# jwwangchn/BONAI

Measured on AMD Instinct MI355X. Metric: training img/s at 1024x1024 LOFT R50-FPN, higher is better.
Workload: dtype bf16; 1 GPU; LOFT R50-FPN + FOA, 8x1024x1024 synthetic tiles per GPU (BASELINE configs[1]), 80 gt/img, full train step (fwd+losses+bwd+allreduce+clip+SGD), random-init weights, RoI heads at the load of a trained RPN (first proposals = jittered gt boxes); global_batch=8, per_gpu_batch=8, parallelism=dp1, graph_features=False

## Files before the change

### bonai_amd/csrc/elementwise.hip

```cpp
#include "loft_common.h"
#include "../../include/loft_hip.h"
#include "conv_tap.h"

__device__ __forceinline__ void ld8(const bf16_t* p, float v[8]) {
    uint4 t = *reinterpret_cast<const uint4*>(p);
    unpack8_16(t, v);
}
__device__ __forceinline__ void st8(bf16_t* p, const float v[8]) {
    *reinterpret_cast<uint4*>(p) = pack8_16(v);
}

__device__ __forceinline__ void ld8(const float* p, float v[8]) { ld4(p, v); ld4(p + 4, v + 4); }
__device__ __forceinline__ void st8(float* p, const float v[8]) { st4(p, v); st4(p + 4, v + 4); }

static inline dim3 ew_grid(long nvec) {
    long b = (nvec + 255) / 256;
    if (b > 8192) b = 8192;
    if (b < 1) b = 1;
    return dim3((unsigned)b);
}

__global__ void relu_bwd_kernel(const bf16_t* __restrict__ g, const bf16_t* __restrict__ y, bf16_t* __restrict__ out,
                                long nvec) {
    for (long i = blockIdx.x * (long)blockDim.x + threadIdx.x; i < nvec; i += (long)gridDim.x * blockDim.x) {
// ... 851 lines not shown
                    for (int k = 0; k < 4; ++k) q[k] = (uint32_t)tp[(2 * k) * ldw] | ((uint32_t)tp[(2 * k + 1) * ldw] << 16);
                    *reinterpret_cast<uint4*>(wpt + ((long)t * CinP + c0 + ccl) * CoutP + nn) = make_uint4(q[0], q[1], q[2], q[3]);
                }
            }
        } else if (wpt) {
            const int hsh = ntsh - 1, hp = 1 << hsh;
            for (int i = threadIdx.x; i < RS * 64 * hp; i += 256) {
                const int np = i & (hp - 1), r2 = i >> hsh, ccl = r2 & 63, t = r2 >> 6;
                const int nn = n0 + 2 * np, cc = c0 + ccl;
                if (nn < CoutP && cc < CinP) {
                    const bf16_t* tp = bt + 2 * np * ldw + ccl * RS + t;
                    *reinterpret_cast<uint32_t*>(wpt + ((long)t * CinP + cc) * CoutP + nn) = (uint32_t)tp[0] | ((uint32_t)tp[ldw] << 16);
                }
            }
        }
    }
}
LOFT_EXPORT int loft_fold_pack_multi(const int64_t* desc, int n, int64_t nchunks, void* stream) {
    if (n <= 0 || nchunks <= 0) return 0;
    long blocks = nchunks < 16384 ? nchunks : 16384;
    hipLaunchKernelGGL(fold_pack_multi_kernel, dim3((unsigned)blocks), dim3(256), 0, (hipStream_t)stream, (const long*)desc, n,
                       (long)nchunks);
    LOFT_LAUNCH_CHECK();
    return 0;
}

__global__ __launch_bounds__(256) void transpose_bf16_kernel(const bf16_t* __restrict__ src, bf16_t* __restrict__ dst, int R, int Cc) {
    __shared__ bf16_t t[64][66];
    const int r0 = blockIdx.y * 64, c0 = blockIdx.x * 64;
    for (int i = threadIdx.x; i < 64 * 32; i += 256) {
        const int r = i >> 5, cp = (i & 31) * 2;
        uint32_t v = 0;
        if (r0 + r < R && c0 + cp < Cc) v = *reinterpret_cast<const uint32_t*>(src + (long)(r0 + r) * Cc + c0 + cp);
        t[r][cp] = (bf16_t)(v & 0xffff);
        t[r][cp + 1] = (bf16_t)(v >> 16);
    }
    __syncthreads();
    for (int i = threadIdx.x; i < 64 * 32; i += 256) {
        const int c = i >> 5, rp = (i & 31) * 2;
        if (c0 + c < Cc && r0 + rp < R)
            *reinterpret_cast<uint32_t*>(dst + (long)(c0 + c) * R + r0 + rp) = (uint32_t)t[rp][c] | ((uint32_t)t[rp + 1][c] << 16);
    }
}
LOFT_EXPORT int loft_transpose_bf16(const void* src, void* dst, int R, int Cc, void* stream) {
    if (R <= 0 || Cc <= 0) return 0;
    if ((R & 1) || (Cc & 1)) return (int)hipErrorInvalidValue;
    hipLaunchKernelGGL(transpose_bf16_kernel, dim3(loft_cdiv(Cc, 64), loft_cdiv(R, 64)), dim3(256), 0, (hipStream_t)stream,
                       (const bf16_t*)src, (bf16_t*)dst, R, Cc);
    LOFT_LAUNCH_CHECK();
    return 0;
}

__global__ __launch_bounds__(256) void fold_unpack_bwd_kernel(const float* __restrict__ dwp, const float* __restrict__ db,
                                                              const float* __restrict__ w, const float* __restrict__ gamma,
                                                              const float* __restrict__ mean, const float* __restrict__ var,
                                                              float eps, int Cout, int Cin, int RS, float* __restrict__ dw,
                                                              float* __restrict__ dgamma, float* __restrict__ dbeta, int CoutP,
                                                              int CinP, int accumulate) {
    const int n = blockIdx.x;
    const float rs = gamma ? rsqrtf(var[n] + eps) : 1.f;
    const float scale = gamma ? gamma[n] * rs : 1.f;
    float acc = 0.f;
    const int per = Cin * RS;
    for (int j = threadIdx.x; j < per; j += blockDim.x) {
        const int c = j / RS, t = j - c * RS;
        const float g = dwp[((long)t * CoutP + n) * CinP + c];
        const long wi = (long)n * per + j;
        if (dw) dw[wi] = (accumulate ? dw[wi] : 0.f) + g * scale;
        if (gamma) acc += g * w[wi];
    }
    if (gamma) {
        for (int o = 32; o > 0; o >>= 1) acc += __shfl_down(acc, o, 64);
        __shared__ float part[4];
        if ((threadIdx.x & 63) == 0) part[threadIdx.x >> 6] = acc;
        __syncthreads();
        if (threadIdx.x == 0) {
            const float s = part[0] + part[1] + part[2] + part[3];
            const float dbn = db ? db[n] : 0.f;
            if (dgamma) dgamma[n] = (accumulate ? dgamma[n] : 0.f) + (s * rs - dbn * mean[n] * rs);
            if (dbeta) dbeta[n] = (accumulate ? dbeta[n] : 0.f) + dbn;
        }
    }
}
__global__ __launch_bounds__(256) void fold_unpack_bwd_multi_kernel(const long* __restrict__ desc, int njobs, int lds_floats) {
    const int lo = find_record(desc, njobs, (long)blockIdx.x);
    const long* d = desc + (long)lo * 16;
    const float* dwp = reinterpret_cast<const float*>(d[0]);
    const float* db = reinterpret_cast<const float*>(d[1]);
    const float* w = reinterpret_cast<const float*>(d[2]);
    const float* gamma = reinterpret_cast<const float*>(d[3]);
    const float* mean = reinterpret_cast<const float*>(d[4]);
    const float* var = reinterpret_cast<const float*>(d[5]);
    float* dw = reinterpret_cast<float*>(d[6]);
    float* dgamma = reinterpret_cast<float*>(d[7]);
    float* dbeta = reinterpret_cast<float*>(d[8]);
    const float eps = __int_as_float((int)(d[9] & 0xffffffffl));
    const int nsp = (int)(d[9] >> 32) > 1 ? (int)(d[9] >> 32) : 1;
    const int Cin = (int)d[11], CoutP = (int)d[13], CinP = (int)d[14];
    const bool nmajor = d[12] < 0;
    const int RS = (int)(nmajor ? -d[12] : d[12]);
    const int n = (int)(blockIdx.x - d[15]);
    const long sps = (long)RS * CoutP * CinP;
    auto ld1 = [&](const float* p) {
        float v = *p;
        int q = 1;
        for (; q + 3 < nsp; q += 4) {
            const float u0 = p[q * sps], u1 = p[(q + 1) * sps], u2 = p[(q + 2) * sps], u3 = p[(q + 3) * sps];
            v += (u0 + u1) + (u2 + u3);
        }
        for (; q < nsp; ++q) v += p[q * sps];
        return v;
    };
    auto ld4s = [&](const float* p) {
        float4 v = *reinterpret_cast<const float4*>(p);
        int q = 1;
        for (; q + 3 < nsp; q += 4) {
            const float4 u0 = *reinterpret_cast<const float4*>(p + q * sps), u1 = *reinterpret_cast<const float4*>(p + (q + 1) * sps);
            const float4 u2 = *reinterpret_cast<const float4*>(p + (q + 2) * sps), u3 = *reinterpret_cast<const float4*>(p + (q + 3) * sps);
            v.x += (u0.x + u1.x) + (u2.x + u3.x); v.y += (u0.y + u1.y) + (u2.y + u3.y);
            v.z += (u0.z + u1.z) + (u2.z + u3.z); v.w += (u0.w + u1.w) + (u2.w + u3.w);
        }
        for (; q < nsp; ++q) {
            const float4 u = *reinterpret_cast<const float4*>(p + q * sps);
            v.x += u.x; v.y += u.y; v.z += u.z; v.w += u.w;
        }
        return v;
    };
    const float rs = gamma ? rsqrtf(var[n] + eps) : 1.f;
    const float scale = gamma ? gamma[n] * rs : 1.f;
    float acc = 0.f;
    const int per = Cin * RS;
    if (nmajor) {
        extern __shared__ float urow[];
        const int CB = min(Cin, lds_floats / RS);
        const unsigned cb_mul = CB == 1 ? 0u : 0xFFFFFFFFu / (unsigned)CB + 1u;
        for (int cb0 = 0; cb0 < Cin; cb0 += CB) {
            const int cbn = min(CB, Cin - cb0), cnt = cbn * RS;
            const bool small = CB * RS < 65536 && cbn == CB;
            __syncthreads();
            for (int j = threadIdx.x; j < cnt; j += blockDim.x) {
                const int t = cbn == 1 ? j : (small ? (int)__umulhi((unsigned)j, cb_mul) : j / cbn), c = j - t * cbn;
                urow[c * RS + t] = ld1(dwp + (long)n * per + (long)t * CinP + cb0 + c);
            }
            __syncthreads();
            for (int j = threadIdx.x; j < cnt; j += blockDim.x) {
                const long wi = (long)n * per + (long)cb0 * RS + j;
                if (dw) dw[wi] += urow[j] * scale;
            }
        }
        if (threadIdx.x == 0 && dbeta && db) dbeta[n] += db[n];
        return;
    }
    if (RS > 1 && per <= lds_floats) {
        extern __shared__ float urow[];
        if ((Cin & 3) == 0 && (CinP & 3) == 0) {
            for (int j = threadIdx.x * 4; j < per; j += blockDim.x * 4) {
                const int t = j / Cin, c = j - t * Cin;
                const float4 v = ld4s(dwp + ((long)t * CoutP + n) * CinP + c);
                urow[c * RS + t] = v.x; urow[(c + 1) * RS + t] = v.y; urow[(c + 2) * RS + t] = v.z; urow[(c + 3) * RS + t] = v.w;
            }
            __syncthreads();
            for (int j = threadIdx.x * 4; j < per; j += blockDim.x * 4) {
                const float4 g = *reinterpret_cast<const float4*>(urow + j);
                const long wi = (long)n * per + j;
                if (dw) {
                    float4 o = *reinterpret_cast<float4*>(dw + wi);
                    o.x += g.x * scale; o.y += g.y * scale; o.z += g.z * scale; o.w += g.w * scale;
                    *reinterpret_cast<float4*>(dw + wi) = o;
                }
                if (gamma) {
                    const float4 ww = *reinterpret_cast<const float4*>(w + wi);
                    acc += g.x * ww.x + g.y * ww.y + g.z * ww.z + g.w * ww.w;
                }
            }
        } else {
            for (int j = threadIdx.x; j < per; j += blockDim.x) {
                const int t = j / Cin, c = j - t * Cin;
                urow[c * RS + t] = ld1(dwp + ((long)t * CoutP + n) * CinP + c);
            }
            __syncthreads();
            for (int j = threadIdx.x; j < per; j += blockDim.x) {
                const float g = urow[j];
                const long wi = (long)n * per + j;
                if (dw) dw[wi] += g * scale;
                if (gamma) acc += g * w[wi];
            }
        }
    } else if (RS == 1 && (Cin & 3) == 0 && (CinP & 3) == 0) {
        for (int j = threadIdx.x * 4; j < per; j += blockDim.x * 4) {
            const float4 g = ld4s(dwp + (long)n * CinP + j);
            const long wi = (long)n * per + j;
            if (dw) {
                float4 o = *reinterpret_cast<float4*>(dw + wi);
                o.x += g.x * scale; o.y += g.y * scale; o.z += g.z * scale; o.w += g.w * scale;
                *reinterpret_cast<float4*>(dw + wi) = o;
            }
            if (gamma) {
                const float4 ww = *reinterpret_cast<const float4*>(w + wi);
                acc += g.x * ww.x + g.y * ww.y + g.z * ww.z + g.w * ww.w;
            }
        }
    } else
    for (int j = threadIdx.x; j < per; j += blockDim.x) {
        const int c = j / RS, t = j - c * RS;
        const float g = ld1(dwp + ((long)t * CoutP + n) * CinP + c);
        const long wi = (long)n * per + j;
        if (dw) dw[wi] += g * scale;
        if (gamma) acc += g * w[wi];
    }
    if (gamma) {
        for (int o = 32; o > 0; o >>= 1) acc += __shfl_down(acc, o, 64);
        __shared__ float part[4];
        if ((threadIdx.x & 63) == 0) part[threadIdx.x >> 6] = acc;
        __syncthreads();
        if (threadIdx.x == 0) {
            const float s = part[0] + part[1] + part[2] + part[3];
            const float dbn = db ? db[n] : 0.f;
            if (dgamma) dgamma[n] += s * rs - dbn * mean[n] * rs;
            if (dbeta) dbeta[n] += dbn;
        }
    } else if (threadIdx.x == 0 && dbeta && db) {
        dbeta[n] += db[n];
    }
}
LOFT_EXPORT int loft_fold_unpack_bwd_multi(const int64_t* desc, int njobs, int64_t nblocks, int lds_floats, void* stream) {
    if (njobs <= 0 || nblocks <= 0) return 0;
    if (lds_floats < 0 || lds_floats > 16384) return (int)hipErrorInvalidValue;
    hipLaunchKernelGGL(fold_unpack_bwd_multi_kernel, dim3((unsigned)nblocks), dim3(256), (size_t)lds_floats * 4, (hipStream_t)stream,
                       (const long*)desc, njobs, lds_floats);
    LOFT_LAUNCH_CHECK();
    return 0;
}
LOFT_EXPORT int loft_fold_unpack_bwd(const float* dwp, const float* db, const float* w, const float* gamma, const float* mean,
                                     const float* var, float eps, int Cout, int Cin, int RS, float* dw, float* dgamma,
                                     float* dbeta, int CoutP, int CinP, int accumulate, void* stream) {
    if (Cout <= 0) return 0;
    if (CoutP < Cout || CinP < Cin) return (int)hipErrorInvalidValue;
    hipLaunchKernelGGL(fold_unpack_bwd_kernel, dim3(Cout), dim3(256), 0, (hipStream_t)stream, dwp, db, w, gamma, mean, var, eps,
                       Cout, Cin, RS, dw, dgamma, dbeta, CoutP, CinP, accumulate);
    LOFT_LAUNCH_CHECK();
    return 0;
}

template <typename T, int V> struct NhbIO;
template <> struct NhbIO<bf16_t, 4> {
    static __device__ __forceinline__ void ld(const bf16_t* p, float* v) { ld4(p, v); }
    static __device__ __forceinline__ void st(bf16_t* p, const float* v) { st4(p, v); }
};
template <> struct NhbIO<bf16_t, 8> {
    static __device__ __forceinline__ void ld(const bf16_t* p, float* v) { ld8(p, v); }
    static __device__ __forceinline__ void st(bf16_t* p, const float* v) { st8(p, v); }
};
template <> struct NhbIO<float, 4> {
    static __device__ __forceinline__ void ld(const float* p, float* v) {
        const float4 a = *reinterpret_cast<const float4*>(p);
        v[0] = a.x; v[1] = a.y; v[2] = a.z; v[3] = a.w;
    }
    static __device__ __forceinline__ void st(float* p, const float* v) { *reinterpret_cast<float4*>(p) = make_float4(v[0], v[1], v[2], v[3]); }
};

template <int NOUT, int V, typename XT = bf16_t>
__global__ __launch_bounds__(256) void narrow_head_bwd_kernel(const float* __restrict__ g, int gs, const XT* __restrict__ x,
                                                              const float* __restrict__ w, long M, int Cin, int relu_in,
                                                              XT* __restrict__ gx, float* __restrict__ dw,
                                                              float* __restrict__ db) {
    const int cg = Cin / V;
    const int ppi = 256 / cg > 0 ? 256 / cg : 1;
    const int tid = threadIdx.x;
    const int col = tid % cg, sub = tid / cg;
    const bool act = sub < ppi;
    const int c0 = col * V;
    float wr[NOUT][V], acc[NOUT][V], bacc[NOUT];
#pragma unroll
    for (int n = 0; n < NOUT; ++n) {
#pragma unroll
        for (int q = 0; q < V; ++q) { wr[n][q] = w[(long)n * Cin + c0 + q]; acc[n][q] = 0.f; }
        bacc[n] = 0.f;
    }
    if (act) {
        constexpr int UN = 4;
        const long step = ppi;
        const long per_blk = ((M + gridDim.x - 1) / gridDim.x + (long)ppi * UN - 1) / ((long)ppi * UN) * ((long)ppi * UN);
        const long m_beg = (long)blockIdx.x * per_blk, m_end = m_beg + per_blk < M ? m_beg + per_blk : M;
        for (long m0 = m_beg + sub; m0 < m_end; m0 += step * UN) {
            float xv[UN][V], gv[UN][NOUT];
#pragma unroll
            for (int u = 0; u < UN; ++u) {
                const long m = m0 + u * step;
                if (m < m_end) {
                    NhbIO<XT, V>::ld(x + m * Cin + c0, xv[u]);
#pragma unroll
                    for (int n = 0; n < NOUT; ++n) gv[u][n] = g[m * gs + n];
                } else {
#pragma unroll
                    for (int q = 0; q < V; ++q) xv[u][q] = 0.f;
#pragma unroll
                    for (int n = 0; n < NOUT; ++n) gv[u][n] = 0.f;
                }
            }
#pragma unroll
            for (int u = 0; u < UN; ++u) {
                const long m = m0 + u * step;
                float o[V];
#pragma unroll
                for (int q = 0; q < V; ++q) o[q] = 0.f;
// ... 183 lines not shown
```

### bonai_amd/debug.py

```python
import contextlib
import os

SWITCHES = {
    'no_side_stream': 'mask / bbox branches, the RPN proposal chain and the backbone weight gradients all on the main stream '
                      '(the mode of bench.py\'s roofline instrumentation)',
    'no_bbox_side_stream': 'the bbox head on the main stream (the mask branch keeps its side stream)',
    'no_rpn_side_stream': 'the RPN proposal chain (sort, decode, NMS) on the main stream',
    'no_rpn_target_prefetch': 'RPN anchor assignment + sampling after the RPN convs on the main stream, not beside the backbone',
    'no_rpn_loss_stream': 'the RPN losses (and with them the sparse RPN backward) on the main stream',
    'no_wgrad_stream': 'backbone weight-gradient launches on the data-gradient stream',
    'unpack_stream': 'the batched weight-gradient unpack launches (descriptor upload + loft_fold_unpack_bwd_multi) on a stream of their '
                     'own instead of on the main stream between the data-gradient kernels (round 6: measured, not the default)',
    'no_prepack': 'BN fold + operand packing per conv per step instead of one launch per step (kernels.PrepackRegistry)',
    'no_unpack_queue': 'one loft_fold_unpack_bwd launch per conv instead of the batched unpack (kernels.UnpackQueue)',
    'no_grad_sink': 'gradients returned to autograd and accumulated by it, not deposited in the arena by the kernels',
    'no_leaf_sink': 'narrow heads and the sparse RPN backward return their parameter gradients to autograd (per-parameter accumulation '
                    'launches) instead of depositing them through the unpack queue (nn._queue_param_grads)',
    'no_head_fusion': 'narrow 1x1 heads (RPN objectness + deltas, mask logits) as launches of their own instead of in the producing '
                      'conv\'s epilogue (loft_conv_tap_bf16_head)',
    'no_grad_join': 'autograd sums the two data gradients of a backbone stage output (next stage + FPN lateral) with an elementwise add '
                    'instead of the residual block taking the lateral\'s deposit as its data-gradient residual (nn.JOIN)',
    'no_deconv_fusion': 'the mask head\'s 2x2 deconvolution as four parity launches instead of one launch whose four channel tiles are '
                        'the four taps (loft_deconv2x2_bf16: the input tile read once)',
    'no_zero_pool': 'torch.zeros / torch.empty per accumulation buffer instead of the step\'s pre-zeroed / scratch slabs',
    'no_feat_hub': 'autograd sums the RPN / RoI-extractor gradients of the FPN maps (no shared per-level gradient map)',
    'no_block_fusion': 'one autograd node per conv of a residual block instead of nn.res_block',
    'no_linear_fn': 'Linear layers through the generic conv node',
    'no_bneck_fusion': 'the frozen / inference 64-plane bottleneck as three (four) tap-conv launches instead of conv1 + the fused tail '
                       '(loft_bneck_tail_bf16: 3x3 + 1x1 expansion + shortcut + ReLU in one launch)',
    'no_pair_fusion': 'the last 1x1 of bottleneck k and the first 1x1 of bottleneck k+1 (layer2 / layer3) as two launches each way instead '
                      'of one (loft_bneck_pair_bf16: the block output is written once and not re-read as the next conv1\'s operand)',
    'wgrad_no_patch': 'the tap weight-gradient kernel for 64-channel high-resolution layers (no patch kernel)',
    'roi_fp32_bwd': 'RoIAlign backward into fp32 maps + a cast',
    'roi_sort': 'RoIAlign forward workgroups in (image, level, row strip) launch order for lists of >= 256 RoIs (loft_roi_order; '
                'measured neutral on the step, not shipped)',
    'no_roi_sort': 'list (sampling) order even where kernels.ROI_FWD_SORT_MIN asks for the launch order',
    'narrow_mfma_bwd': 'narrow (<= 8 output) heads backward as padded MFMA GEMMs',
}


class _Switches:
    __slots__ = tuple(SWITCHES)

    def __init__(self):
        for k in SWITCHES:
            setattr(self, k, bool(os.environ.get('LOFT_' + k.upper())))

    def active(self):
        return sorted(k for k in SWITCHES if getattr(self, k))

    @contextlib.contextmanager
    def override(self, **kw):
        prev = {k: getattr(self, k) for k in kw}
        try:
            for k, v in kw.items():
                setattr(self, k, bool(v))
            yield self
        finally:
            for k, v in prev.items():
                setattr(self, k, v)


DBG = _Switches()
```

### bonai_amd/engine.py

```python
import os

import torch
import torch.distributed as dist

from . import kernels as K
from .debug import DBG


class FlatArena:

    def __init__(self, model):
        self.params = [p for p in model.parameters() if p.requires_grad]
        dev = self.params[0].device
        order = list(reversed(self.params))
        self.offsets, off = {}, 0
        for p in order:
            self.offsets[id(p)] = off
            off += (p.numel() + 7) // 8 * 8
        self.numel = off
        self.data = torch.zeros(off, dtype=torch.float32, device=dev)
        self.grad = torch.zeros(off, dtype=torch.float32, device=dev)
        self.momentum = torch.zeros(off, dtype=torch.float32, device=dev)
        for p in order:
            o = self.offsets[id(p)]
# ... 144 lines not shown
        for raw, st in producers.items():
            ev = self._events.get((bi, raw))
            if ev is None:
                ev = self._events[(bi, raw)] = torch.cuda.Event()
            ev.record(st)
            self.stream.wait_event(ev)
        with torch.cuda.stream(self.stream):
            self.works.append(dist.all_reduce(view, async_op=True))

    def finish(self):
        if not self.enabled:
            return
        while self._next < len(self.buckets):
            self._launch(self._next)
            self._next += 1
        if self.on_gpu and self.measure:
            e0 = torch.cuda.Event(enable_timing=True)
            e0.record(torch.cuda.current_stream())
        if self.on_gpu:
            if self.works and dist.get_backend() == 'nccl':
                with torch.cuda.stream(self.stream):
                    self.works[-1].wait()
            else:
                for w in self.works:
                    w.wait()
            if self.measure:
                e1 = torch.cuda.Event(enable_timing=True)
                e1.record(self.stream)
                self.exposed.append((e0, e1))
            torch.cuda.current_stream().wait_stream(self.stream)
        else:
            for w in self.works:
                w.wait()
        self._prune()

    def _prune(self):
        if not self.prune_hooks or self.capturing:
            return
        for p in self.arena.order:
            k = id(p)
            if k in self._via_sink:
                if k in self._hooks:
                    self._sunk_streak[k] += 1
                    if self._sunk_streak[k] >= self.PRUNE_AFTER:
                        self._hooks.pop(k).remove()
            elif k in self._hooks:
                self._sunk_streak[k] = 0
            elif k not in self._seen:
                self._arm(p)

    def exposed_ms(self):
        ev, self.exposed = self.exposed, []
        if not ev:
            return None
        return sum(max(0.0, a.elapsed_time(b)) for a, b in ev) / len(ev)


def step_lr(base_lr, it, epoch, warmup_iters=300, warmup_ratio=0.001, steps=(16, 22), gamma=0.1, step=None):
    if step is not None:
        steps = step
    lr = base_lr * gamma ** sum(epoch >= s for s in steps)
    if it < warmup_iters:
        k = (1 - it / warmup_iters) * (1 - warmup_ratio)
        lr = lr * (1 - k)
    return lr


class Trainer:
    def __init__(self, model, lr=0.005, momentum=0.9, weight_decay=1e-4, max_norm=35.0, bucket_bytes=25 << 20,
                 loss_scale=1.0, graph_features=False):
        self.model = model
        self.graph_features = bool(graph_features)
        self._fgraphs = None
        self._unpack_stream = None
        self._steps_run = 0
        self.lr, self.mu, self.wd, self.max_norm = lr, momentum, weight_decay, max_norm
        self.loss_scale = float(loss_scale)
        self.arena = FlatArena(model)
        self.reducer = BucketedAllReduce(self.arena, bucket_bytes)
        self.world = dist.get_world_size() if self.reducer.enabled else 1
        self.gnorm_sq = torch.zeros(1, dtype=torch.float32, device=self.arena.data.device)
        self.iter = 0
        self.prepack = K.PrepackRegistry()
        self._sink = self.reducer._sink if self.reducer.enabled else (lambda p: None)

    def _graph_step_setup(self, img):
        from .graphs import FeatureGraphs
        fg = self._fgraphs
        if fg is None:
            fg = self._fgraphs = FeatureGraphs(self)
        if fg.ready and fg.validate() is not None:
            import warnings
            warnings.warn(f'hipGraphs of backbone + neck dropped and recaptured: {fg.stale}', RuntimeWarning)
        if not fg.ready and fg.failed is None and self._steps_run >= 2 and self.prepack.order:
            self.reducer.capturing = True
            try:
                fg.capture(img)
            except Exception as e:
                import warnings
                fg.failed = f'{type(e).__name__}: {e}'
                warnings.warn(f'hipGraph capture of backbone + neck failed, the trainer stays on eager launches: {fg.failed}',
                              RuntimeWarning)
            finally:
                self.reducer.capturing = False
        if fg.ready:
            self.model.feat_provider = fg.provider

    def optimizer_state_dict(self):
        a = self.arena
        state, idx = {}, {}
        for i, p in enumerate(self.model.parameters()):
            idx[id(p)] = i
        if self.iter > 0:
            for p in a.params:
                o = a.offsets[id(p)]
                state[idx[id(p)]] = dict(momentum_buffer=a.momentum[o:o + p.numel()].view(p.shape).detach().cpu().clone())
        group = dict(lr=self.lr, momentum=self.mu, dampening=0, weight_decay=self.wd, nesterov=False,
                     params=list(range(len(idx))))
        return dict(state=state, param_groups=[group], iter=self.iter, sampler_calls=int(K._SAMPLE_CALLS[0]))

    def load_optimizer_state(self, sd):
        a = self.arena
        params = list(self.model.parameters())
        state = sd.get('state', {})
        groups = sd.get('param_groups')
        if groups and sum(len(g.get('params', ())) for g in groups) != len(params):
            raise RuntimeError(f"optimizer state covers {sum(len(g['params']) for g in groups)} parameters, the model has "
                               f'{len(params)}: it was written for a different model')
        todo = []
        for i, st in state.items():
            if not 0 <= int(i) < len(params):
                raise RuntimeError(f'optimizer state index {i} outside the model\'s {len(params)} parameters')
            p = params[int(i)]
            buf = st.get('momentum_buffer')
            if buf is None:
                continue
            if tuple(buf.shape) != tuple(p.shape):
                raise RuntimeError(f'optimizer state {i}: momentum_buffer {tuple(buf.shape)} does not fit parameter '
                                   f'{tuple(p.shape)} (parameter order differs from the checkpoint\'s)')
            if id(p) in a.offsets:
                todo.append((a.offsets[id(p)], p.numel(), buf))
        for o, n, buf in todo:
            a.momentum[o:o + n].copy_(buf.reshape(-1).to(a.momentum.device))
        self.iter = int(sd.get('iter', self.iter))
        if 'sampler_calls' in sd:
            K._SAMPLE_CALLS[0] = int(sd['sampler_calls'])

    def train_step(self, data, lr=None):
        self.arena.grad.zero_()
        self.arena.rebind_grads()
        self.reducer.begin()
        for p in self.arena.params:
            p._loft_pending = 0
            p._loft_sunk = False
        from . import nn as F2
        prev_pp, prev_wpl = F2.PREPACK, K.WEIGHT_PLANES
        if self.arena.data.is_cuda and not DBG.no_prepack:
            F2.PREPACK = self.prepack
            K.WEIGHT_PLANES = self.prepack.wplanes
            self.prepack.run(self.iter)
        prev_hub = F2.HUB_ENABLED
        F2.HUB_ENABLED = self.arena.data.is_cuda and not DBG.no_feat_hub
        F2.JOIN = {} if (self.arena.data.is_cuda and not DBG.no_grad_join) else None
        F2.PAIR_G.clear()
        if self.graph_features and self.arena.data.is_cuda and K.PROFILE is None and F2.PREPACK is not None \
                and hasattr(self.model, 'extract_feat'):
            self._graph_step_setup(data['img'])
        try:
            out = self.model.train_step(data)
        except BaseException:
            F2.JOIN = None
            K.WEIGHT_PLANES = prev_wpl
            raise
        finally:
            F2.PREPACK = prev_pp
            F2.HUB_ENABLED = prev_hub
            if self.graph_features:
                self.model.feat_provider = None
        prev, F2.GRAD_SINK = F2.GRAD_SINK, (self._sink if self.arena.data.is_cuda and not DBG.no_grad_sink else None)
        if self.arena.data.is_cuda and not DBG.no_zero_pool:
            K.zero_pool_begin(self.arena.data.device)
        if F2.GRAD_SINK is not None and not DBG.no_unpack_queue:
            ustream = None
            if DBG.unpack_stream and not DBG.no_side_stream:
                if getattr(self, '_unpack_stream', None) is None:
                    self._unpack_stream = torch.cuda.Stream()
                ustream = self._unpack_stream
            lim = int(os.environ.get('LOFT_UNPACK_LIMIT', '0')) or (24 if self.reducer.enabled else 48)
            note = self.reducer.note_queued if (self.reducer.enabled and os.environ.get('LOFT_NO_NOTE_FLUSH') != '1') else None
            F2.UNPACK_Q = K.UnpackQueue(limit=lim, note=note, stream=ustream)
            if not DBG.no_side_stream and not DBG.no_wgrad_stream:
                if getattr(self, '_wgrad_stream', None) is None:
                    self._wgrad_stream = torch.cuda.Stream()
                F2.WGRAD_STREAM = self._wgrad_stream
        try:
            (out['loss'] if self.loss_scale == 1.0 else out['loss'] * self.loss_scale).backward()
            if F2.UNPACK_Q is not None:
                F2.UNPACK_Q.flush()
        finally:
            if F2.UNPACK_Q is not None:
                F2.UNPACK_Q.join()
            F2.UNPACK_Q = None
            F2.WGRAD_STREAM = None
            F2.GRAD_SINK = prev
            F2.HUB = None
            F2.JOIN = None
            K.WEIGHT_PLANES = prev_wpl
            K.zero_pool_end()
        self.reducer.finish()
        self.gnorm_sq.zero_()
        K.sumsq_(self.arena.grad, self.gnorm_sq)
        K.sgd_momentum_(self.arena.data, self.arena.grad, self.arena.momentum, self.gnorm_sq, self.max_norm,
                        self.lr if lr is None else lr, self.mu, self.wd, grad_scale=1.0 / (self.world * self.loss_scale))
        self.iter += 1
        self._steps_run += 1
        return out
```

### bonai_amd/kernels.py

```python
import ctypes
import os

import numpy as np
import torch

from . import lib as L
from .debug import DBG as _DBG

c_int, c_int64, c_float, c_void_p = ctypes.c_int, ctypes.c_int64, ctypes.c_float, ctypes.c_void_p


def h2d(values, dtype, device):
    t = torch.from_numpy(values).to(dtype) if isinstance(values, np.ndarray) else torch.tensor(values, dtype=dtype)
    if torch.device(device).type != 'cuda':
        return t.to(device)
    if H2D_KEEP is not None:
        global _H2D_STREAM
        for _ in range(64):
            if _H2D_STREAM is None:
                _H2D_STREAM = torch.cuda.Stream()
            with torch.cuda.stream(_H2D_STREAM):
                if not torch.cuda.is_current_stream_capturing():
                    break
            _H2D_STREAM = None
# ... 1894 lines not shown
    nv = nval.contiguous().view(torch.uint8) if nval.dtype == torch.bool else nval.contiguous()
    tab = torch.empty(4, B, dtype=torch.int32, device=dev)
    L.check(lib.loft_roi_sample_offsets(L.ptr(pv), L.ptr(nv), B, P, Q, L.ptr(tab), L.stream()), 'loft_roi_sample_offsets')
    Mx, Nx = B * (P + Q), B * P
    out = dict(rois=torch.zeros(Mx, 5, device=dev), labels=torch.empty(Mx, dtype=torch.int64, device=dev),
               label_weights=torch.empty(Mx, device=dev), bbox_targets=torch.empty(Mx, 4, device=dev),
               bbox_weights=torch.empty(Mx, 4, device=dev), pos_rois=torch.empty(Nx, 5, device=dev),
               pos_b=torch.empty(Nx, dtype=torch.int64, device=dev), pos_gt_i=torch.empty(Nx, dtype=torch.int64, device=dev),
               pos_sel=torch.empty(Nx, dtype=torch.int64, device=dev))
    if Mx > 0:
        L.check(lib.loft_roi_sample_targets(L.ptr(cand.float().contiguous()), Ncand, L.ptr(gt_inds.contiguous()),
                                            L.ptr(gts.float().contiguous()), L.ptr(gt_labels.contiguous()), int(gts.shape[1]),
                                            L.ptr(pidx.contiguous()), L.ptr(nidx.contiguous()), P, Q, B, L.ptr(tab[0]), L.ptr(tab[1]),
                                            L.ptr(tab[2]), L.ptr(tab[3]), int(num_classes), L.arr(c_float, list(means)),
                                            L.arr(c_float, list(stds)), L.ptr(out['rois']), L.ptr(out['labels']),
                                            L.ptr(out['label_weights']), L.ptr(out['bbox_targets']), L.ptr(out['bbox_weights']),
                                            L.ptr(out['pos_rois']), L.ptr(out['pos_b']), L.ptr(out['pos_gt_i']), L.ptr(out['pos_sel']),
                                            L.stream()), 'loft_roi_sample_targets')
    host = torch.empty(2, B, dtype=torch.int32, pin_memory=True)
    host.copy_(tab[:2], non_blocking=True)
    ev = torch.cuda.Event()
    ev.record()
    return _RoiTargets(out, host, ev, B, Mx if num_expected is None else min(Mx, B * int(num_expected)))


def roi_sample_targets(cand, gt_inds, gts, gt_labels, pidx, pval, nidx, nval, num_classes, means, stds):
    return roi_sample_targets_begin(cand, gt_inds, gts, gt_labels, pidx, pval, nidx, nval, num_classes, means, stds).finish()


_SAMPLE_CALLS = [0]


def random_sample(gt_inds, num, max_pos, mode='random'):
    lib = L.load()
    L.dev_check(gt_inds)
    gt_inds = gt_inds.contiguous()
    if gt_inds.dtype != torch.int64:
        raise L.LoftHipError(f'gt_inds must be int64, got {gt_inds.dtype}')
    B, N = gt_inds.shape
    P, Q = min(int(max_pos), N), min(int(num), N)
    dev = gt_inds.device
    pidx = torch.empty(B, P, dtype=torch.int64, device=dev)
    nidx = torch.empty(B, Q, dtype=torch.int64, device=dev)
    pval = torch.empty(B, P, dtype=torch.uint8, device=dev)
    nval = torch.empty(B, Q, dtype=torch.uint8, device=dev)
    _SAMPLE_CALLS[0] += 1
    seed = (torch.initial_seed() * 6364136223846793005 + _SAMPLE_CALLS[0] * 1442695040888963407) & 0xFFFFFFFFFFFFFFFF
    if B > 0 and N > 0:
        ws = torch.empty(B * ((N + 15) // 16 * 16), dtype=torch.uint8, device=dev)
        L.check(lib.loft_random_sample(L.ptr(gt_inds), B, N, int(num), int(max_pos), 0 if mode == 'first' else 1,
                                       ctypes.c_uint64(seed), L.ptr(pidx), L.ptr(pval), L.ptr(nidx), L.ptr(nval), L.ptr(ws),
                                       L.stream()), 'loft_random_sample')
    return pidx, pval.view(torch.bool), nidx, nval.view(torch.bool)


def sampled_avg_factor(pos_valid, neg_valid):
    lib = L.load()
    L.dev_check(pos_valid, neg_valid)
    pv, nv = pos_valid.contiguous().view(torch.uint8), neg_valid.contiguous().view(torch.uint8)
    out = torch.empty(1, dtype=torch.float32, device=pv.device)
    L.check(lib.loft_sampled_avg_factor(L.ptr(pv), L.ptr(nv), int(pv.shape[0]), int(pv.shape[1]), int(nv.shape[1]), L.ptr(out),
                                        L.stream()), 'loft_sampled_avg_factor')
    return out


def narrow_head_bwd(g, x, w, relu_in=False, need_gx=True, need_dw=True, need_db=True):
    lib = L.load()
    L.dev_check(g, x, w)
    x = _nhwc(x)
    g = g.float().contiguous(memory_format=torch.channels_last)
    N, Cin, H, W = x.shape
    Cout = w.shape[0]
    w2 = w.reshape(Cout, Cin).float().contiguous()
    f32 = x.dtype == torch.float32
    gx = empty_nhwc(N, Cin, H, W, torch.float32 if f32 else L.act16(), x.device) if need_gx else None
    dw = pooled_zeros((Cout, Cin), x.device) if need_dw else None
    db = pooled_zeros((Cout,), x.device) if need_db else None
    fn = lib.loft_narrow_head_bwd_f32 if f32 else lib.loft_narrow_head_bwd
    L.check(fn(L.ptr(g), int(g.shape[1]), L.ptr(x), L.ptr(w2), c_int64(N * H * W), Cin, Cout, int(relu_in),
               L.ptr(gx), L.ptr(dw), L.ptr(db), L.stream()), 'loft_narrow_head_bwd')
    return gx, dw, db


class UnpackQueue:

    def __init__(self, limit=48, note=None, stream=None):
        self.limit = limit
        self.note = note
        self.jobs, self.done = [], []
        self.main = torch.cuda.current_stream() if torch.cuda.is_available() else None
        self.main_raw = L.stream().value if self.main is not None else None
        self.home = stream if stream is not None else self.main
        self.home_raw = self.home.cuda_stream if stream is not None else self.main_raw
        self.dedicated = stream is not None
        self.events = []
        self.main_jobs = False
        self.keep = []
        self._targets = set()

    def add(self, dwp, db, w, bn, eps, slots, on_done=(), flat_chw=None, nsplit=1, params=()):
        tgt = slots[0].data_ptr() if slots[0] is not None else None
        if tgt is not None:
            if tgt in self._targets:
                if os.environ.get('LOFT_DEBUG_TARGETS'):
                    print('unpack queue: slot used twice in one batch ->', tuple(w.shape), 'jobs pending', len(self.jobs), flush=True)
                self.flush()
            self._targets.add(tgt)
        self.jobs.append((dwp, db, w, bn, float(eps), slots, flat_chw, int(nsplit)))
        if self.home is not None:
            raw = L.stream().value
            if raw == self.home_raw:
                pass
            elif self.dedicated and raw == self.main_raw:
                self.main_jobs = True
            else:
                ev = torch.cuda.Event()
                ev.record()
                self.events.append(ev)
                if not self.dedicated:
                    for t in (dwp, db):
                        if t is not None:
                            t.record_stream(self.home)
            if self.dedicated:
                self.keep.append((dwp, db))
        self.done.extend(on_done)
        if len(self.jobs) >= self.limit or (self.note is not None and self.note(params)):
            self.flush()

    def join(self, stream=None):
        if self.dedicated:
            (stream or self.main).wait_stream(self.home)
        self.keep = []

    def flush(self):
        if self.home is not None and L.stream().value != self.home_raw:
            if self.main_jobs:
                ev = torch.cuda.Event()
                ev.record(self.main)
                self.events.append(ev)
                self.main_jobs = False
            with torch.cuda.stream(self.home):
                return self.flush()
        for ev in self.events:
            self.home.wait_event(ev)
        self.events = []
        if self.jobs:
            import struct
            rows, blk = [], 0
            p = lambda t: 0 if t is None else t.data_ptr()
            for dwp, db, w, bn, eps, (dw, dg, dbeta), flat, nsplit in self.jobs:
                if flat is not None:
                    Cout, Cin, RS = w.shape[0], flat[0], -(flat[1] * flat[2])
                    coutp, cinp = Cout, Cin
                else:
                    Cout, Cin = w.shape[0], w.shape[1]
                    RS = w.shape[2] * w.shape[3] if w.dim() == 4 else 1
                    coutp, cinp = dwp.shape[-2], dwp.shape[-1]
                g, _, m, v = bn if bn is not None else (None, None, None, None)
                rows.append([p(dwp), p(db), p(w), p(g), p(m), p(v), p(dw), p(dg), p(dbeta),
                             (struct.unpack('<I', struct.pack('<f', eps))[0]) | (nsplit << 32), Cout, Cin, RS, coutp, cinp, blk])
                blk += Cout
            desc = h2d(rows, torch.int64, self.jobs[0][2].device)
            lds = max([min(r[11], 64) * abs(r[12]) if r[12] < 0 else r[11] * r[12] for r in rows
                       if r[12] < 0 or (r[12] > 1 and r[11] * r[12] <= 16384)], default=0)
            if lds > 16384:
                raise L.LoftHipError(f'fold_unpack_bwd_multi: a record needs {lds} floats of LDS')
            L.check(L.load().loft_fold_unpack_bwd_multi(L.ptr(desc), len(rows), c_int64(blk), int(lds), L.stream()),
                    'loft_fold_unpack_bwd_multi')
            self.jobs = []
            self._targets = set()
        done, self.done = self.done, []
        for f in done:
            f()


def fold_unpack_bwd(dwp, db, w, bn=None, eps=1e-5, need_dw=True, out=None):
    lib = L.load()
    w = w.contiguous()
    Cout, Cin, R, S = w.shape
    dev = w.device
    g = m = v = dg = dbeta = None
    if out is not None:
        dw, dg, dbeta = out
        if bn is not None:
            g, _, m, v = [t.contiguous() for t in bn]
    else:
        dw = torch.empty_like(w) if need_dw else None
        if bn is not None:
            g, _, m, v = [t.contiguous() for t in bn]
            dg = torch.empty(Cout, dtype=torch.float32, device=dev)
            dbeta = torch.empty(Cout, dtype=torch.float32, device=dev)
    L.check(lib.loft_fold_unpack_bwd(L.ptr(dwp), L.ptr(db), L.ptr(w), L.ptr(g), L.ptr(m), L.ptr(v), c_float(eps), Cout, Cin,
                                     R * S, L.ptr(dw), L.ptr(dg), L.ptr(dbeta), dwp.shape[-2], dwp.shape[-1], int(out is not None),
                                     L.stream()),
            'loft_fold_unpack_bwd')
    return dw, dg, dbeta
```

Baseline: 231.6 img/s.

## Store first weight-gradient deposit instead of zeroing the whole gradient arena

Adds a DepositPlan that learns which gradient-arena slots the batched unpack kernel writes each step. On later steps it zeroes only the gaps, and the kernel's first deposit into a covered slot overwrites instead of read-modify-write accumulating. This removes the full arena memset and one read per weight gradient element. It also vectorises the n-major unpack path with float4 loads and stores. The cost is host-side bookkeeping per deposit and a correctness dependence on the deposit order staying the same between steps.

```diff
diff --git a/bonai_amd/csrc/elementwise.hip b/bonai_amd/csrc/elementwise.hip
--- a/bonai_amd/csrc/elementwise.hip
+++ b/bonai_amd/csrc/elementwise.hip
@@ -957,6 +957,7 @@
         }
     }
 }
+constexpr int UNPACK_STORE_W = 60, UNPACK_STORE_G = 61, UNPACK_STORE_B = 62;
 __global__ __launch_bounds__(256) void fold_unpack_bwd_multi_kernel(const long* __restrict__ desc, int njobs, int lds_floats) {
     const int lo = find_record(desc, njobs, (long)blockIdx.x);
     const long* d = desc + (long)lo * 16;
@@ -970,7 +971,9 @@
     float* dgamma = reinterpret_cast<float*>(d[7]);
     float* dbeta = reinterpret_cast<float*>(d[8]);
     const float eps = __int_as_float((int)(d[9] & 0xffffffffl));
-    const int nsp = (int)(d[9] >> 32) > 1 ? (int)(d[9] >> 32) : 1;
+    const int nsp_raw = (int)((d[9] >> 32) & 0xffffff);
+    const int nsp = nsp_raw > 1 ? nsp_raw : 1;
+    const bool st_w = (d[9] >> UNPACK_STORE_W) & 1, st_g = (d[9] >> UNPACK_STORE_G) & 1, st_b = (d[9] >> UNPACK_STORE_B) & 1;
     const int Cin = (int)d[11], CoutP = (int)d[13], CinP = (int)d[14];
     const bool nmajor = d[12] < 0;
     const int RS = (int)(nmajor ? -d[12] : d[12]);
@@ -1003,16 +1006,45 @@
     };
     const float rs = gamma ? rsqrtf(var[n] + eps) : 1.f;
     const float scale = gamma ? gamma[n] * rs : 1.f;
+    auto dep1 = [&](float* p, float g) {
+        float o = 0.f;
+        if (!st_w) o = *p;
+        *p = o + g * scale;
+    };
+    auto dep4 = [&](float* p, const float4 g) {
+        float4 o = make_float4(0.f, 0.f, 0.f, 0.f);
+        if (!st_w) o = *reinterpret_cast<const float4*>(p);
+        o.x += g.x * scale; o.y += g.y * scale; o.z += g.z * scale; o.w += g.w * scale;
+        *reinterpret_cast<float4*>(p) = o;
+    };
     float acc = 0.f;
     const int per = Cin * RS;
     if (nmajor) {
         extern __shared__ float urow[];
-        const int CB = min(Cin, lds_floats / RS);
+        const int cb_fit = min(Cin, lds_floats / RS);
+        const int CB = cb_fit >= 4 ? cb_fit & ~3 : cb_fit;
         const unsigned cb_mul = CB == 1 ? 0u : 0xFFFFFFFFu / (unsigned)CB + 1u;
+        const bool v4 = (Cin & 3) == 0 && (CinP & 3) == 0 && (CB & 3) == 0 &&
+                        ((reinterpret_cast<uintptr_t>(dwp) | reinterpret_cast<uintptr_t>(dw)) & 15) == 0;
         for (int cb0 = 0; cb0 < Cin; cb0 += CB) {
             const int cbn = min(CB, Cin - cb0), cnt = cbn * RS;
             const bool small = CB * RS < 65536 && cbn == CB;
             __syncthreads();
+            if (v4) {
+                const int q = cbn >> 2, cnt4 = q * RS;
+                for (int j = threadIdx.x; j < cnt4; j += blockDim.x) {
+                    const int t = j / q, c = (j - t * q) << 2;
+                    const float4 v = ld4s(dwp + (long)n * per + (long)t * CinP + cb0 + c);
+                    urow[c * RS + t] = v.x; urow[(c + 1) * RS + t] = v.y; urow[(c + 2) * RS + t] = v.z; urow[(c + 3) * RS + t] = v.w;
+                }
+                __syncthreads();
+                for (int j = threadIdx.x * 4; j < cnt; j += blockDim.x * 4) {
+                    const float4 g = *reinterpret_cast<const float4*>(urow + j);
+                    const long wi = (long)n * per + (long)cb0 * RS + j;
+                    if (dw) dep4(dw + wi, g);
+                }
+                continue;
+            }
             for (int j = threadIdx.x; j < cnt; j += blockDim.x) {
                 const int t = cbn == 1 ? j : (small ? (int)__umulhi((unsigned)j, cb_mul) : j / cbn), c = j - t * cbn;
                 urow[c * RS + t] = ld1(dwp + (long)n * per + (long)t * CinP + cb0 + c);
@@ -1020,10 +1052,10 @@
             __syncthreads();
             for (int j = threadIdx.x; j < cnt; j += blockDim.x) {
                 const long wi = (long)n * per + (long)cb0 * RS + j;
-                if (dw) dw[wi] += urow[j] * scale;
-            }
-        }
-        if (threadIdx.x == 0 && dbeta && db) dbeta[n] += db[n];
+                if (dw) dep1(dw + wi, urow[j]);
+            }
+        }
+        if (threadIdx.x == 0 && dbeta && db) dbeta[n] = (st_b ? 0.f : dbeta[n]) + db[n];
         return;
     }
     if (RS > 1 && per <= lds_floats) {
@@ -1038,11 +1070,7 @@
             for (int j = threadIdx.x * 4; j < per; j += blockDim.x * 4) {
                 const float4 g = *reinterpret_cast<const float4*>(urow + j);
                 const long wi = (long)n * per + j;
-                if (dw) {
-                    float4 o = *reinterpret_cast<float4*>(dw + wi);
-                    o.x += g.x * scale; o.y += g.y * scale; o.z += g.z * scale; o.w += g.w * scale;
-                    *reinterpret_cast<float4*>(dw + wi) = o;
-                }
+                if (dw) dep4(dw + wi, g);
                 if (gamma) {
                     const float4 ww = *reinterpret_cast<const float4*>(w + wi);
                     acc += g.x * ww.x + g.y * ww.y + g.z * ww.z + g.w * ww.w;
@@ -1057,7 +1085,7 @@
             for (int j = threadIdx.x; j < per; j += blockDim.x) {
                 const float g = urow[j];
                 const long wi = (long)n * per + j;
-                if (dw) dw[wi] += g * scale;
+                if (dw) dep1(dw + wi, g);
                 if (gamma) acc += g * w[wi];
             }
         }
@@ -1065,11 +1093,7 @@
         for (int j = threadIdx.x * 4; j < per; j += blockDim.x * 4) {
             const float4 g = ld4s(dwp + (long)n * CinP + j);
             const long wi = (long)n * per + j;
-            if (dw) {
-                float4 o = *reinterpret_cast<float4*>(dw + wi);
-                o.x += g.x * scale; o.y += g.y * scale; o.z += g.z * scale; o.w += g.w * scale;
-                *reinterpret_cast<float4*>(dw + wi) = o;
-            }
+            if (dw) dep4(dw + wi, g);
             if (gamma) {
                 const float4 ww = *reinterpret_cast<const float4*>(w + wi);
                 acc += g.x * ww.x + g.y * ww.y + g.z * ww.z + g.w * ww.w;
@@ -1080,7 +1104,7 @@
         const int c = j / RS, t = j - c * RS;
         const float g = ld1(dwp + ((long)t * CoutP + n) * CinP + c);
         const long wi = (long)n * per + j;
-        if (dw) dw[wi] += g * scale;
+        if (dw) dep1(dw + wi, g);
         if (gamma) acc += g * w[wi];
     }
     if (gamma) {
@@ -1091,11 +1115,11 @@
         if (threadIdx.x == 0) {
             const float s = part[0] + part[1] + part[2] + part[3];
             const float dbn = db ? db[n] : 0.f;
-            if (dgamma) dgamma[n] += s * rs - dbn * mean[n] * rs;
-            if (dbeta) dbeta[n] += dbn;
+            if (dgamma) dgamma[n] = (st_g ? 0.f : dgamma[n]) + (s * rs - dbn * mean[n] * rs);
+            if (dbeta) dbeta[n] = (st_b ? 0.f : dbeta[n]) + dbn;
         }
     } else if (threadIdx.x == 0 && dbeta && db) {
-        dbeta[n] += db[n];
+        dbeta[n] = (st_b ? 0.f : dbeta[n]) + db[n];
     }
 }
 LOFT_EXPORT int loft_fold_unpack_bwd_multi(const int64_t* desc, int njobs, int64_t nblocks, int lds_floats, void* stream) {
diff --git a/bonai_amd/debug.py b/bonai_amd/debug.py
--- a/bonai_amd/debug.py
+++ b/bonai_amd/debug.py
@@ -22,6 +22,8 @@
                     'instead of the residual block taking the lateral\'s deposit as its data-gradient residual (nn.JOIN)',
     'no_deconv_fusion': 'the mask head\'s 2x2 deconvolution as four parity launches instead of one launch whose four channel tiles are '
                         'the four taps (loft_deconv2x2_bf16: the input tile read once)',
+    'no_deposit_store': 'the whole gradient arena zeroed every step and every weight-gradient deposit accumulated into it, instead of '
+                        'the batched unpack storing its first deposit of a step into slots left unzeroed (kernels.DepositPlan)',
     'no_zero_pool': 'torch.zeros / torch.empty per accumulation buffer instead of the step\'s pre-zeroed / scratch slabs',
     'no_feat_hub': 'autograd sums the RPN / RoI-extractor gradients of the FPN maps (no shared per-level gradient map)',
     'no_block_fusion': 'one autograd node per conv of a residual block instead of nn.res_block',
diff --git a/bonai_amd/engine.py b/bonai_amd/engine.py
--- a/bonai_amd/engine.py
+++ b/bonai_amd/engine.py
@@ -250,6 +250,7 @@
         self.gnorm_sq = torch.zeros(1, dtype=torch.float32, device=self.arena.data.device)
         self.iter = 0
         self.prepack = K.PrepackRegistry()
+        self.deposit = K.DepositPlan(self.arena.grad)
         self._sink = self.reducer._sink if self.reducer.enabled else (lambda p: None)
 
     def _graph_step_setup(self, img):
@@ -315,13 +316,15 @@
             K._SAMPLE_CALLS[0] = int(sd['sampler_calls'])
 
     def train_step(self, data, lr=None):
-        self.arena.grad.zero_()
+        from . import nn as F2
+        sink_on = self.arena.data.is_cuda and not DBG.no_grad_sink and not DBG.no_unpack_queue
+        self.deposit.begin(sink_on and not DBG.no_deposit_store and not self.graph_features,
+                           (tuple(DBG.active()), K.PROFILE is not None, F2.GRAD_SINK is not None))
         self.arena.rebind_grads()
         self.reducer.begin()
         for p in self.arena.params:
             p._loft_pending = 0
             p._loft_sunk = False
-        from . import nn as F2
         prev_pp, prev_wpl = F2.PREPACK, K.WEIGHT_PLANES
         if self.arena.data.is_cuda and not DBG.no_prepack:
             F2.PREPACK = self.prepack
@@ -356,7 +359,7 @@
                 ustream = self._unpack_stream
             lim = int(os.environ.get('LOFT_UNPACK_LIMIT', '0')) or (24 if self.reducer.enabled else 48)
             note = self.reducer.note_queued if (self.reducer.enabled and os.environ.get('LOFT_NO_NOTE_FLUSH') != '1') else None
-            F2.UNPACK_Q = K.UnpackQueue(limit=lim, note=note, stream=ustream)
+            F2.UNPACK_Q = K.UnpackQueue(limit=lim, note=note, stream=ustream, plan=self.deposit if self.deposit.learning else None)
             if not DBG.no_side_stream and not DBG.no_wgrad_stream:
                 if getattr(self, '_wgrad_stream', None) is None:
                     self._wgrad_stream = torch.cuda.Stream()
@@ -375,6 +378,7 @@
             F2.JOIN = None
             K.WEIGHT_PLANES = prev_wpl
             K.zero_pool_end()
+        self.deposit.finish()
         self.reducer.finish()
         self.gnorm_sq.zero_()
         K.sumsq_(self.arena.grad, self.gnorm_sq)
diff --git a/bonai_amd/kernels.py b/bonai_amd/kernels.py
--- a/bonai_amd/kernels.py
+++ b/bonai_amd/kernels.py
@@ -2000,10 +2000,78 @@
     return gx, dw, db
 
 
+class DepositPlan:
+    MAX_GAPS = 24
+
+    def __init__(self, grad):
+        self.grad = grad
+        self.base, self.numel = grad.data_ptr(), grad.numel()
+        self.covered = {}
+        self.sig = None
+        self.gaps = None
+        self.active = False
+        self.learning = False
+        self.dirty = False
+        self.deposited, self.new = set(), {}
+
+    def begin(self, use, sig):
+        if sig != self.sig or self.dirty:
+            self.covered, self.gaps, self.sig = {}, None, sig
+        self.deposited, self.new = set(), {}
+        self.learning = bool(use)
+        self.active = bool(use) and bool(self.covered)
+        self.dirty = True
+        if not self.active:
+            self.grad.zero_()
+            return
+        if self.gaps is None:
+            self.gaps = self._gaps()
+        if len(self.gaps) > self.MAX_GAPS:
+            self.grad.zero_()
+        else:
+            for v in self.gaps:
+                v.zero_()
+
+    def _gaps(self):
+        out, pos = [], 0
+        for off, n in sorted(self.covered.values()) + [(self.numel, 0)]:
+            if off > pos and not (off - pos < 8 and off % 8 == 0 and pos > 0):
+                out.append(self.grad[pos:off])
+            pos = max(pos, off + n)
+        return out
+
+    def first(self, t):
+        if t is None:
+            return False
+        a = t.data_ptr()
+        if a in self.deposited:
+            return False
+        off = (a - self.base) // 4
+        if not (0 <= off and off + t.numel() <= self.numel and (a - self.base) % 4 == 0 and t.is_contiguous()):
+            return False
+        self.deposited.add(a)
+        if a in self.covered:
+            return self.active
+        if self.learning:
+            self.new[a] = (off, t.numel())
+        return False
+
+    def finish(self):
+        if self.active:
+            for a, (off, n) in self.covered.items():
+                if a not in self.deposited:
+                    self.grad[off:off + n].zero_()
+        if self.new:
+            self.covered.update(self.new)
+            self.gaps = None
+        self.dirty = False
+
+
 class UnpackQueue:
 
-    def __init__(self, limit=48, note=None, stream=None):
+    def __init__(self, limit=48, note=None, stream=None, plan=None):
         self.limit = limit
+        self.plan = plan
         self.note = note
         self.jobs, self.done = [], []
         self.main = torch.cuda.current_stream() if torch.cuda.is_available() else None
@@ -2017,13 +2085,13 @@
         self._targets = set()
 
     def add(self, dwp, db, w, bn, eps, slots, on_done=(), flat_chw=None, nsplit=1, params=()):
-        tgt = slots[0].data_ptr() if slots[0] is not None else None
-        if tgt is not None:
-            if tgt in self._targets:
+        tgts = [t.data_ptr() for t in slots if t is not None]
+        if tgts:
+            if any(t in self._targets for t in tgts):
                 if os.environ.get('LOFT_DEBUG_TARGETS'):
                     print('unpack queue: slot used twice in one batch ->', tuple(w.shape), 'jobs pending', len(self.jobs), flush=True)
                 self.flush()
-            self._targets.add(tgt)
+            self._targets.update(tgts)
         self.jobs.append((dwp, db, w, bn, float(eps), slots, flat_chw, int(nsplit)))
         if self.home is not None:
             raw = L.stream().value
@@ -2075,8 +2143,11 @@
                     RS = w.shape[2] * w.shape[3] if w.dim() == 4 else 1
                     coutp, cinp = dwp.shape[-2], dwp.shape[-1]
                 g, _, m, v = bn if bn is not None else (None, None, None, None)
+                store = 0
+                if self.plan is not None:
+                    store = (int(self.plan.first(dw)) << 60) | (int(self.plan.first(dg)) << 61) | (int(self.plan.first(dbeta)) << 62)
                 rows.append([p(dwp), p(db), p(w), p(g), p(m), p(v), p(dw), p(dg), p(dbeta),
-                             (struct.unpack('<I', struct.pack('<f', eps))[0]) | (nsplit << 32), Cout, Cin, RS, coutp, cinp, blk])
+                             (struct.unpack('<I', struct.pack('<f', eps))[0]) | (nsplit << 32) | store, Cout, Cin, RS, coutp, cinp, blk])
                 blk += Cout
             desc = h2d(rows, torch.int64, self.jobs[0][2].device)
             lds = max([min(r[11], 64) * abs(r[12]) if r[12] < 0 else r[11] * r[12] for r in rows
```

Measured after the change: 232.5 img/s (median of 2 runs). Within noise of the previous version (+0.4%).
